# theouterlimitz/Audio-Mastering-Engine

Measured on NVIDIA B200. Metric: audio-sec mastered/sec (x realtime), higher is better.
Workload: dtype f64

## Files before the change

### audio_mastering_engine_b200/csrc/ame.cu

```cuda
#include <algorithm>
#include <cmath>
#include <cstdarg>
#include <cstdio>
#include <cstring>
#include <dlfcn.h>
#include <mutex>
#include <string>
#include <vector>

#include "ame_kernels.cuh"

using namespace ame;

namespace {

thread_local std::string g_err;

int fail(int code, const char *fmt, ...) {
    char buf[512];
    va_list ap;
    va_start(ap, fmt);
    vsnprintf(buf, sizeof buf, fmt, ap);
    va_end(ap);
    g_err = buf;
// ... 114 lines not shown
    std::vector<Slot> slots;
    double *d_energy = nullptr;
    int *d_chain_stats = nullptr;
    long long *d_hist = nullptr;
    int *d_hist_st = nullptr;
    int *d_peak = nullptr;
    unsigned *d_tp = nullptr;
    int *d_lim_stats = nullptr;
    int lim_guess = -1;
    ame_track_result *d_results = nullptr;
    KwJob *d_meter_kw = nullptr;
    GainJob *d_meter_peak = nullptr;
    int32_t *d_meter_tracks = nullptr;
    TrackDev *d_meter_tdev = nullptr;
    double *d_meter_energy = nullptr;
    int *d_meter_sp = nullptr;
    unsigned *d_meter_tp = nullptr;
    ame_loudness *d_loud_out = nullptr;
    ame_loudness *d_loud_any = nullptr;
    cudaStream_t s_in = nullptr, s_out = nullptr;
    std::vector<cudaEvent_t> ev_in, ev_run;
    std::vector<cudaEvent_t> ev_meter;
    bool timing = false;
    int t_step = -1, t_wave = 0;
    std::vector<cudaEvent_t> t_ev;
    std::vector<char> t_used;
    std::vector<cudaEvent_t> tl_ev;
    int tl_waves = 0;
};

namespace {

inline bool t_on(const ame_plan *p) {
    return p->timing && p->t_step >= 0 && p->t_step < kMaxTimedSteps && p->t_wave < kMaxTimedWaves;
}
inline size_t t_slot(const ame_plan *p, int kernel) {
    return ((size_t)p->t_step * kMaxTimedWaves + p->t_wave) * AME_N_KERNELS + kernel;
}
inline void t_begin(ame_plan *p, int kernel, cudaStream_t s) {
    if (t_on(p)) cudaEventRecord(p->t_ev[t_slot(p, kernel) * 2], s);
}
inline void t_end(ame_plan *p, int kernel, cudaStream_t s) {
    if (t_on(p)) {
        cudaEventRecord(p->t_ev[t_slot(p, kernel) * 2 + 1], s);
        p->t_used[t_slot(p, kernel)] = 1;
    }
}

int plan_alloc(ame_plan *p, void **ptr, size_t bytes) {
    *ptr = nullptr;
    if (bytes == 0) return AME_OK;
    cudaError_t e = dev_alloc(ptr, bytes);
    if (e != cudaSuccess) {
        *ptr = nullptr;
        return fail(AME_E_NOMEM, "device allocation of %zu bytes failed: %s", bytes, cudaGetErrorString(e));
    }
    p->allocs.push_back(*ptr);
    return AME_OK;
}

int dmalloc(ame_plan *p, void **ptr, size_t bytes) {
    const int rc = plan_alloc(p, ptr, bytes);
    if (rc == AME_OK) p->ws_bytes += bytes;
    return rc;
}

template <class T>
int upload(ame_plan *p, T **dptr, const std::vector<T> &v) {
    if (int rc = plan_alloc(p, (void **)dptr, v.size() * sizeof(T))) return rc;
    if (!v.empty()) CU(cudaMemcpy(*dptr, v.data(), v.size() * sizeof(T), cudaMemcpyHostToDevice));
    return AME_OK;
}

#define LAUNCH_CHECK(p)                                                                            \
    do {                                                                                           \
        cudaError_t e_ = cudaGetLastError();                                                       \
        if (e_ != cudaSuccess) return fail(AME_E_CUDA, "kernel launch failed: %s (%s:%d)", cudaGetErrorString(e_), __FILE__, __LINE__); \
        ++(p)->launches;                                                                           \
    } while (0)

int check_warmth(const ame_plan *p) {
    for (int t = 0; t < p->n_tracks; ++t)
        if (p->tracks[t].flags & AME_F_WARMTH) {
            const int l = p->tracks[t].warm_lut;
            if (l < 0 || l >= p->n_luts) return fail(AME_E_INVALID, "track %d needs warmth table %d but %d are set", t, l, p->n_luts);
        }
    return AME_OK;
}

struct Bufs {
    const int16_t *in = nullptr;
    int16_t *pre = nullptr, *bands = nullptr, *out = nullptr;
    uint16_t *rms = nullptr, *list = nullptr;
    int *tile_cnt = nullptr, *n_flagged = nullptr;
    GrpRec *grp = nullptr;
    double *att = nullptr;
    int64_t *hist = nullptr;
    int16_t *norm = nullptr;
    long long *lim_last = nullptr;
    LimStore lim_in{}, lim_out{};
    int *lim_need = nullptr;
};

Bufs slot_bufs(ame_plan *p, const Wave &w, const int16_t *d_in, int16_t *d_out) {
    const Slot &sl = p->slots[w.slot];
    Bufs b;
    b.in = d_in; b.out = d_out;
    b.pre = sl.pre - 2 * w.frame_lo;
    b.bands = sl.bands; b.rms = sl.rms; b.list = sl.list; b.tile_cnt = sl.tile_cnt; b.n_flagged = sl.n_flagged;
    b.grp = sl.grp; b.att = sl.att;
    b.norm = sl.norm ? sl.norm - 2 * w.frame_lo : nullptr;
    b.lim_last = sl.lim_last; b.lim_in = sl.lim_in; b.lim_out = sl.lim_out; b.lim_need = sl.lim_need;
    b.hist = (int64_t *)p->d_hist;
    return b;
}

int run_eq(ame_plan *p, const Wave &w, const int16_t *d_in, int16_t *d_pre, cudaStream_t s) {
    if (!w.eq.n) return AME_OK;
    t_begin(p, S_EQ, s);
    if (p->precision == 1)
        k_eq_f32<<<(w.eq.n + 127) / 128, 128, 0, s>>>(p->d_eq_jobs + w.eq.lo, w.eq.n, p->d_tracks, p->d_luts, d_in, d_pre);
    else
        k_eq<<<(w.eq.n + kEqBlock - 1) / kEqBlock, kEqBlock, 0, s>>>(p->d_eq_jobs + w.eq.lo, w.eq.n, p->d_tracks, p->d_luts, d_in, d_pre);
    LAUNCH_CHECK(p);
    t_end(p, S_EQ, s);
    return AME_OK;
}

int run_split(ame_plan *p, const Wave &w, const int16_t *d_pre, int16_t *d_bands, cudaStream_t s) {
    if (!w.split.n) return AME_OK;
    t_begin(p, S_SPLIT, s);
    if (w.xover_uni)
        k_band_split<true><<<(w.split.n + 127) / 128, 128, 0, s>>>(w.xover, p->d_split_jobs + w.split.lo, w.split.n, p->d_tracks, p->d_mb_delta,
                                                                   d_pre, d_bands, p->mb_frames);
    else
        k_band_split<false><<<(w.split.n + 127) / 128, 128, 0, s>>>(w.xover, p->d_split_jobs + w.split.lo, w.split.n, p->d_tracks, p->d_mb_delta,
                                                                    d_pre, d_bands, p->mb_frames);
    LAUNCH_CHECK(p);
    t_end(p, S_SPLIT, s);
    return AME_OK;
}

int chain_lanes(const ame_plan *p, int n_chains) {
    if (p->chain_warps < 0) return 1;
    if (p->chain_warps > 0) return 32 * p->chain_warps;
    if (n_chains * 2 <= p->n_sm) return 256;
    return (n_chains >= p->n_sm && p->slots.size() > 1) ? 64 : 128;
}

int run_compress(ame_plan *p, const Wave &w, const Bufs &b, cudaStream_t s) {
    if (!w.chain.n) return AME_OK;
    t_begin(p, S_FLAG, s);
    int *tile_base = b.tile_cnt + std::max(p->slot_tiles, 1);
    k_window_flag<<<w.wf.n, kWfThreads, 0, s>>>(p->d_wf_jobs + w.wf.lo, b.bands, b.rms, b.tile_cnt, b.grp);
    LAUNCH_CHECK(p);
    k_tile_prefix<<<w.chain.n, kWfThreads, 0, s>>>(p->d_chain_jobs + w.chain.lo, b.tile_cnt, tile_base, b.n_flagged);
    LAUNCH_CHECK(p);
    k_compact<<<(w.wf.n + kWfThreads / 32 - 1) / (kWfThreads / 32), kWfThreads, 0, s>>>(p->d_wf_jobs + w.wf.lo, w.wf.n, b.rms, b.tile_cnt,
                                                                                          tile_base, b.list, b.grp);
    LAUNCH_CHECK(p);
    t_end(p, S_FLAG, s);
    t_begin(p, S_CHAIN, s);
    const int lanes = chain_lanes(p, w.chain.n);
    k_att_chain<<<w.chain.n, std::max(lanes, 32), 0, s>>>(p->d_chain_jobs + w.chain.lo, b.list, b.n_flagged, p->d_tables, b.att, p->mb_frames,
                                            lanes, p->d_chain_stats + 2 * (size_t)w.chain.lo);
    LAUNCH_CHECK(p);
    t_end(p, S_CHAIN, s);
    t_begin(p, S_APPLY, s);
    k_compress_apply<<<(unsigned)((w.seg_hi - w.seg_lo + 3) / 4), 128, 0, s>>>(p->d_mb_chunks + w.mb_chunks.lo, w.mb_chunks.n, w.seg_lo, w.seg_hi,
                                                                                b.bands, b.grp, b.att, b.pre, p->mb_frames);
    LAUNCH_CHECK(p);
    t_end(p, S_APPLY, s);
    return AME_OK;
}

int run_hist(ame_plan *p, const Wave &w, const int16_t *d_pre, int64_t *d_hist, cudaStream_t s) {
    const int nt = w.track_hi - w.track_lo;
    if (nt <= 0) return AME_OK;
    CU(cudaMemsetAsync(p->d_peak + w.track_lo, 0, (size_t)nt * 4, s));
    if (w.kw.n) {
        t_begin(p, S_KW, s);
        if (w.kw_uni)
            k_kweight_energy<true><<<(w.kw.n + 127) / 128, 128, 0, s>>>(w.kw_cfg, p->d_kw_jobs + w.kw.lo, w.kw.n, p->d_tracks, p->d_tdev, d_pre,
                                                                        p->d_energy, p->d_peak);
        else
            k_kweight_energy<false><<<(w.kw.n + 127) / 128, 128, 0, s>>>(w.kw_cfg, p->d_kw_jobs + w.kw.lo, w.kw.n, p->d_tracks, p->d_tdev, d_pre,
                                                                         p->d_energy, p->d_peak);
        LAUNCH_CHECK(p);
        t_end(p, S_KW, s);
    }
    t_begin(p, S_TAIL, s);
    k_tail_peak<<<nt, 128, 0, s>>>(p->d_tracks, p->d_tdev, w.track_lo, w.track_hi, d_pre, p->d_peak);
    LAUNCH_CHECK(p);
    t_end(p, S_TAIL, s);
    CU(cudaMemsetAsync(p->d_tp + w.track_lo, 0, (size_t)nt * 4, s));
    if (w.true_peak && w.gain.n) {
        t_begin(p, S_TP, s);
        k_true_peak<<<w.gain.n, 256, 0, s>>>(p->d_gain_jobs + w.gain.lo, p->d_tracks, d_pre, p->d_tp);
        LAUNCH_CHECK(p);
        t_end(p, S_TP, s);
    }
    t_begin(p, S_HIST, s);
    k_block_hist<<<nt, 256, 0, s>>>(p->d_tdev, w.track_lo, p->d_energy, (long long *)d_hist, p->d_hist_st);
    LAUNCH_CHECK(p);
    t_end(p, S_HIST, s);
    return AME_OK;
}

int run_apply(ame_plan *p, const Wave &w, const int16_t *d_pre, int16_t *d_out, const Bufs &b, cudaStream_t s) {
    int16_t *d_norm = b.norm;
    long long *lim_last = b.lim_last;
    if (!w.gain.n) return AME_OK;
    t_begin(p, S_GAIN, s);
    if (w.limiter) CU(cudaMemsetAsync(lim_last, 0xff, (size_t)w.lim.n * sizeof(long long), s));
    k_apply_gain<<<w.gain.n, 256, 0, s>>>(p->d_gain_jobs + w.gain.lo, p->d_results, p->d_tracks, p->d_tdev, d_pre, d_out, d_norm, lim_last);
    LAUNCH_CHECK(p);
    t_end(p, S_GAIN, s);
    if (w.limiter) {
        t_begin(p, S_LIM, s);
        const GainJob *gj = p->d_lim_jobs + w.lim.lo;
        constexpr int kLimRounds = 2;
        int cap = 64;
        while (cap < p->lim_keep + 2) cap *= 2;
        const size_t smem = lim_smem_bytes(cap);
        for (int round = 0; round <= kLimRounds; ++round) {
            if (round == 0) {
                k_limiter<<<w.lim.n, 256, smem, s>>>(gj, w.lim.n, lim_last, p->d_tracks, d_norm, d_out, b.lim_in, b.lim_out, b.lim_need, 0, cap, p->lim_guess);
                LAUNCH_CHECK(p);
            }
            k_limiter<<<w.lim.n, 32, smem, s>>>(gj, w.lim.n, lim_last, p->d_tracks, d_norm, d_out, b.lim_in, b.lim_out, b.lim_need, round, cap, p->lim_guess);
            LAUNCH_CHECK(p);
            k_lim_verify<<<(w.lim.n + 3) / 4, 128, 0, s>>>(gj, w.lim.n, p->d_tracks, b.lim_in, b.lim_out, b.lim_need,
                                                             p->d_lim_stats + round);
            LAUNCH_CHECK(p);
        }
        k_lim_fallback<<<w.lim.n, 32, smem, s>>>(gj, w.lim.n, p->d_tracks, d_norm, d_out, b.lim_in, b.lim_out, b.lim_need, cap);
        LAUNCH_CHECK(p);
        t_end(p, S_LIM, s);
    }
    return AME_OK;
}

int run_gain(ame_plan *p, const Wave &w, const int16_t *d_pre, const int64_t *d_hist, int16_t *d_out, const Bufs &b, cudaStream_t s) {
    const int nt = w.track_hi - w.track_lo;
    if (nt <= 0) return AME_OK;
    t_begin(p, S_FIN, s);
    k_finalize<<<nt, 128, 0, s>>>(p->d_tracks, w.track_lo, w.track_hi, (const long long *)d_hist, p->d_hist_st, p->d_peak,
                                             p->d_tp, p->d_results);
    LAUNCH_CHECK(p);
    t_end(p, S_FIN, s);
    return run_apply(p, w, d_pre, d_out, b, s);
}

int run_meter(ame_plan *p, const Wave &w, const int16_t *buf, ame_loudness *res, cudaStream_t s) {
    if (!w.meter_tracks.n) return AME_OK;
    const int nt = w.track_hi - w.track_lo;
    CU(cudaMemsetAsync(p->d_meter_sp + w.track_lo, 0, (size_t)nt * 4, s));
    CU(cudaMemsetAsync(p->d_meter_tp + w.track_lo, 0, (size_t)nt * 4, s));
    if (w.meter_kw.n) {
        if (w.kw_uni)
            k_kweight_energy<true><<<(w.meter_kw.n + 127) / 128, 128, 0, s>>>(w.kw_cfg, p->d_meter_kw + w.meter_kw.lo, w.meter_kw.n, p->d_tracks,
                                                                              p->d_meter_tdev, buf, p->d_meter_energy, p->d_meter_sp);
        else
            k_kweight_energy<false><<<(w.meter_kw.n + 127) / 128, 128, 0, s>>>(w.kw_cfg, p->d_meter_kw + w.meter_kw.lo, w.meter_kw.n, p->d_tracks,
                                                                               p->d_meter_tdev, buf, p->d_meter_energy, p->d_meter_sp);
        LAUNCH_CHECK(p);
    }
    if (w.meter_peak.n) {
        k_meter_peak<<<w.meter_peak.n, 256, 0, s>>>(p->d_meter_peak + w.meter_peak.lo, p->d_tracks, buf, p->d_meter_tp, p->d_meter_sp);
        LAUNCH_CHECK(p);
    }
    k_meter_finalize<<<w.meter_tracks.n, 256, 0, s>>>(p->d_meter_tracks + w.meter_tracks.lo, p->d_tracks, p->d_meter_tdev, p->d_meter_energy,
                                                      p->d_meter_sp, p->d_meter_tp, res);
    LAUNCH_CHECK(p);
    return AME_OK;
}

int run_measure(ame_plan *p, const Wave &w, const Bufs &b, cudaStream_t s) {
    int rc;
    if ((rc = run_eq(p, w, b.in, b.pre, s))) return rc;
    if ((rc = run_split(p, w, b.pre, b.bands, s))) return rc;
    if ((rc = run_compress(p, w, b, s))) return rc;
    return run_hist(p, w, b.pre, b.hist, s);
}

int run_chain_of_stages(ame_plan *p, const Wave &w, const Bufs &b, cudaStream_t s) {
    int rc = run_measure(p, w, b, s);
    if (rc) return rc;
    return run_gain(p, w, b.pre, b.hist, b.out, b, s);
}

int drain(ame_plan *p, int rc) {
    (void)p;
    if (rc != AME_OK) cudaDeviceSynchronize();
    return rc;
}

}

extern "C" {

int ame_abi_version(void) { return AME_ABI_VERSION; }
size_t ame_sizeof_track_params(void) { return sizeof(ame_track_params); }
size_t ame_sizeof_track_result(void) { return sizeof(ame_track_result); }
size_t ame_sizeof_plan_options(void) { return sizeof(ame_plan_options); }
size_t ame_sizeof_loudness(void) { return sizeof(ame_loudness); }
const char *ame_last_error(void) { return g_err.c_str(); }
// ... 615 lines not shown
```

### audio_mastering_engine_b200/csrc/ame_kernels.cuh

```cuda
#pragma once
#include <cuda_runtime.h>
#include <stdint.h>
#include "ame_layout.h"

namespace ame {

constexpr unsigned kFull = 0xffffffffu;

__constant__ double c_hist_bounds[1001];
__constant__ double c_hist_energy[1000];

__device__ __forceinline__ uint4 ldg16(const uint4 *p) { return __ldg(p); }

__device__ __forceinline__ double bq_step(const ame_biquad &c, double &z0, double &z1, double x) {
    double y = fma(c.b0, x, z0);
    z0 = fma(-c.a1, y, fma(c.b1, x, z1));
    z1 = fma(-c.a2, y, c.b2 * x);
    return y;
}

__device__ __forceinline__ double i16_to_f64(int x) {
    return __hiloint2double(0x43300000, (int)(0x80000000u ^ (unsigned)x)) - 4503601774854144.0;
}

// ... 144 lines not shown
        }
        if (widen) {
            const float mid = __fmul_rn(__fadd_rn(yl, yr), 0.5f);
            const float side = __fmul_rn(__fmul_rn(__fsub_rn(yl, yr), 0.5f), wfac);
            yl = __fadd_rn(mid, side);
            yr = __fsub_rn(mid, side);
        }
        return pack16(to_pcm_f32(yl), to_pcm_f32(yr));
    };

    const uint4 *src = reinterpret_cast<const uint4 *>(in) + (g0f >> 2);
    uint4 *dst = reinterpret_cast<uint4 *>(pre) + (g0f >> 2);
    uint4 cur = ldg16(src), nxt = make_uint4(0, 0, 0, 0);
    if (g0f + 0 < job.chunk_begin) cur.x = 0;
    if (g0f + 1 < job.chunk_begin) cur.y = 0;
    if (g0f + 2 < job.chunk_begin) cur.z = 0;
    if (n_it > 1) nxt = ldg16(src + 1);
    double lutL[4] = {0, 0, 0, 0}, lutR[4] = {0, 0, 0, 0};
    auto fetch_lut = [&](const uint4 &q, double *l, double *r) {
        const uint32_t w[4] = {q.x, q.y, q.z, q.w};
#pragma unroll
        for (int k = 0; k < 4; ++k) {
            l[k] = __ldg(lut + (int)(int16_t)(w[k] & 0xffffu));
            r[k] = __ldg(lut + (int)(int16_t)(w[k] >> 16));
        }
    };
    if (WARM) fetch_lut(cur, lutL, lutR);
    constexpr int LAG = (SKEW && MASK != 0) ? 1 : 0;
    for (int it = 0; it < n_it + LAG; ++it) {
        uint4 nn = nxt;
        if (it + 2 < n_it) nn = ldg16(src + it + 2);
        double nL[4] = {0, 0, 0, 0}, nR[4] = {0, 0, 0, 0};
        if (WARM) fetch_lut(nxt, nL, nR);
        const int64_t g = g0f + 4 * (int64_t)(it - LAG);
        const uint32_t w[4] = {cur.x, cur.y, cur.z, cur.w};
        uint32_t o[4];
#pragma unroll
        for (int k = 0; k < 4; ++k) o[k] = frame(w[k], lutL[k], lutR[k]);
        if (it < LAG) {
        } else if (g >= job.tile_begin && g + 4 <= f_hi) {
            dst[it - LAG] = make_uint4(o[0], o[1], o[2], o[3]);
        } else {
#pragma unroll
            for (int k = 0; k < 4; ++k)
                if (g + k >= job.tile_begin && g + k < f_hi) reinterpret_cast<uint32_t *>(dst + it - LAG)[k] = o[k];
        }
        cur = nxt; nxt = nn;
#pragma unroll
        for (int k = 0; k < 4; ++k) { lutL[k] = nL[k]; lutR[k] = nR[k]; }
    }
}

#define AME_EQ_KERNEL(NAME, F, SK)                                                                                  \
__global__ void __launch_bounds__(256, 1)                                                                          \
NAME(const TileJob *__restrict__ jobs, int n_jobs, const ame_track_params *__restrict__ tracks,                    \
     const double *__restrict__ luts, const int16_t *__restrict__ in, int16_t *__restrict__ pre) {                 \
    const int j = blockIdx.x * blockDim.x + threadIdx.x;                                                           \
    if (j >= n_jobs) return;                                                                                       \
    const TileJob job = jobs[j];                                                                                   \
    if (job.tile_end <= job.tile_begin) return;                          \
    const ame_track_params *tp = tracks + job.track;                                                               \
    switch (job.variant) {                                                 \
        AME_EQ_CASE(0, F, SK) AME_EQ_CASE(1, F, SK) AME_EQ_CASE(2, F, SK) AME_EQ_CASE(3, F, SK) AME_EQ_CASE(4, F, SK)    \
        AME_EQ_CASE(5, F, SK) AME_EQ_CASE(6, F, SK) AME_EQ_CASE(7, F, SK) AME_EQ_CASE(8, F, SK) AME_EQ_CASE(9, F, SK)    \
        AME_EQ_CASE(10, F, SK) AME_EQ_CASE(11, F, SK) AME_EQ_CASE(12, F, SK) AME_EQ_CASE(13, F, SK) AME_EQ_CASE(14, F, SK) \
        AME_EQ_CASE(15, F, SK)                                                                                     \
    }                                                                                                              \
}
#define AME_EQ_CASE(M, F, SK) case M: eq_tile<M, false, F, SK>(job, tp, luts, in, pre); break; \
                              case M + 16: eq_tile<M, true, F, SK>(job, tp, luts, in, pre); break;
AME_EQ_KERNEL(k_eq, double, false)
AME_EQ_KERNEL(k_eq_f32, float, false)
#undef AME_EQ_CASE
#undef AME_EQ_KERNEL

template <bool UNI>
__global__ void __launch_bounds__(128, 3)
k_band_split(const __grid_constant__ XoverCfg xc, const TileJob *__restrict__ jobs, int n_jobs, const ame_track_params *__restrict__ tracks,
             const int64_t *__restrict__ mb_delta,
             const int16_t *__restrict__ pre, int16_t *__restrict__ bands, int64_t mb_frames) {
    const int j = blockIdx.x * blockDim.x + threadIdx.x;
    if (j >= n_jobs) return;
    const TileJob job = jobs[j];
    const ame_track_params *tp = tracks + job.track;
    const double lb0 = UNI ? xc.lb0 : tp->xlp[0].b0, la10 = UNI ? xc.la10 : tp->xlp[0].a1, la20 = UNI ? xc.la20 : tp->xlp[0].a2,
                 la11 = UNI ? xc.la11 : tp->xlp[1].a1, la21 = UNI ? xc.la21 : tp->xlp[1].a2;
    const double hb0 = UNI ? xc.hb0 : tp->xhp[0].b0, ha10 = UNI ? xc.ha10 : tp->xhp[0].a1, ha20 = UNI ? xc.ha20 : tp->xhp[0].a2,
                 ha11 = UNI ? xc.ha11 : tp->xhp[1].a1, ha21 = UNI ? xc.ha21 : tp->xhp[1].a2;
    const int64_t delta = mb_delta[job.track];
    double zl[8], zr[8];
#pragma unroll
    for (int i = 0; i < 8; ++i) { zl[i] = 0.0; zr[i] = 0.0; }
    int64_t f_lo = job.tile_begin - (int64_t)tp->warm_xover;
    if (f_lo < job.chunk_begin) f_lo = job.chunk_begin;
    const int64_t f_hi = job.tile_end;
    if (f_hi <= f_lo) return;
    const int64_t g0f = f_lo & ~(int64_t)7;
    const int n_it = (int)((f_hi - g0f + 7) >> 3);
    uint32_t *b0 = reinterpret_cast<uint32_t *>(bands) + delta;
    uint32_t *b1 = b0 + mb_frames;
    uint32_t *b2 = b1 + mb_frames;

    auto split = [&](int xm, double *z, int &p0, int &p1, int &p2) {
        const double x = i16_to_unit(xm);
        const double lo = bw_step1<1, double>(la11, la21, z[2], z[3], bw_step<1, double>(lb0, la10, la20, z[0], z[1], x));
        const double hi = bw_step1<-1, double>(ha11, ha21, z[6], z[7], bw_step<-1, double>(hb0, ha10, ha20, z[4], z[5], x));
        const double mid = __dsub_rn(__dsub_rn(x, lo), hi);
        p0 = to_pcm_f64(lo); p1 = to_pcm_f64(mid); p2 = to_pcm_f64(hi);
    };

    const uint4 *src = reinterpret_cast<const uint4 *>(pre) + (g0f >> 2);
    uint4 c0 = ldg16(src), c1 = ldg16(src + 1), n0 = make_uint4(0, 0, 0, 0), n1 = n0;
    {
        uint32_t *cw0 = reinterpret_cast<uint32_t *>(&c0), *cw1 = reinterpret_cast<uint32_t *>(&c1);
#pragma unroll
        for (int k = 0; k < 4; ++k) {
            if (g0f + k < job.chunk_begin) cw0[k] = 0;
            if (g0f + 4 + k < job.chunk_begin) cw1[k] = 0;
        }
    }
    if (n_it > 1) { n0 = ldg16(src + 2); n1 = ldg16(src + 3); }
    for (int it = 0; it < n_it; ++it) {
        uint4 m0 = n0, m1 = n1;
        if (it + 2 < n_it) { m0 = ldg16(src + 2 * it + 4); m1 = ldg16(src + 2 * it + 5); }
        const int64_t g = g0f + 8 * (int64_t)it;
        const uint32_t w[8] = {c0.x, c0.y, c0.z, c0.w, c1.x, c1.y, c1.z, c1.w};
        uint32_t o0[8], o1[8], o2[8];
#pragma unroll
        for (int k = 0; k < 8; ++k) {
            int l0, l1, l2, r0, r1, r2;
            split((int)(int16_t)(w[k] & 0xffffu), zl, l0, l1, l2);
            split((int)(int16_t)(w[k] >> 16), zr, r0, r1, r2);
            o0[k] = pack16(l0, r0); o1[k] = pack16(l1, r1); o2[k] = pack16(l2, r2);
        }
        if (g >= job.tile_begin && g + 8 <= f_hi) {
            uint4 *q0 = reinterpret_cast<uint4 *>(b0 + g), *q1 = reinterpret_cast<uint4 *>(b1 + g), *q2 = reinterpret_cast<uint4 *>(b2 + g);
            q0[0] = make_uint4(o0[0], o0[1], o0[2], o0[3]); q0[1] = make_uint4(o0[4], o0[5], o0[6], o0[7]);
            q1[0] = make_uint4(o1[0], o1[1], o1[2], o1[3]); q1[1] = make_uint4(o1[4], o1[5], o1[6], o1[7]);
            q2[0] = make_uint4(o2[0], o2[1], o2[2], o2[3]); q2[1] = make_uint4(o2[4], o2[5], o2[6], o2[7]);
        } else {
#pragma unroll
            for (int k = 0; k < 8; ++k)
                if (g + k >= job.tile_begin && g + k < f_hi) { b0[g + k] = o0[k]; b1[g + k] = o1[k]; b2[g + k] = o2[k]; }
        }
        c0 = n0; c1 = n1; n0 = m0; n1 = m1;
    }
}

__device__ __forceinline__ unsigned energy_of(uint32_t w) {
    const int l = (int16_t)(w & 0xffffu), r = (int16_t)(w >> 16);
    return (unsigned)(l * l) + (unsigned)(r * r);
}

__device__ __forceinline__ void load8(const uint32_t *__restrict__ p, int64_t idx, int64_t lo, int64_t hi, uint32_t *w) {
    if (idx >= lo && idx + 8 <= hi && ((reinterpret_cast<uintptr_t>(p + idx) & 15) == 0)) {
        const uint4 a = __ldg(reinterpret_cast<const uint4 *>(p + idx));
        const uint4 b = __ldg(reinterpret_cast<const uint4 *>(p + idx) + 1);
        w[0] = a.x; w[1] = a.y; w[2] = a.z; w[3] = a.w; w[4] = b.x; w[5] = b.y; w[6] = b.z; w[7] = b.w;
    } else {
#pragma unroll
        for (int k = 0; k < 8; ++k) w[k] = (idx + k >= lo && idx + k < hi) ? __ldg(p + idx + k) : 0u;
    }
}

__device__ __forceinline__ unsigned isqrt_ratio(unsigned long long s, unsigned n) {
    unsigned r = (unsigned)__fsqrt_rn(__fdividef((float)s, (float)n));
    if ((unsigned long long)r * r * n > s) --r;
    else if ((unsigned long long)(r + 1) * (r + 1) * n <= s) ++r;
    return r;
}

__global__ void __launch_bounds__(kWfThreads)
k_window_flag(const WfJob *__restrict__ jobs, const int16_t *__restrict__ bands, uint16_t *__restrict__ rms,
              int *__restrict__ tile_cnt, GrpRec *__restrict__ grp) {
    __shared__ long long s_scan[kWfThreads / 32];
    __shared__ unsigned long long s_head[kWfThreads / 32];
    __shared__ int s_flag[kWfThreads / 32];
    const WfJob job = jobs[blockIdx.x];
    const uint32_t *bp = reinterpret_cast<const uint32_t *>(bands) + job.plane_off;
    uint16_t *rp = rms + job.plane_off;
    const int64_t n = job.n, t0 = job.tile_begin;
    const int look = job.look;
    const int lane = threadIdx.x & 31, wid = threadIdx.x >> 5;
    const int64_t i0 = t0 + (int64_t)threadIdx.x * 8;
    uint32_t w[8], wo[8];
    load8(bp, i0, 0, n, w);
    load8(bp, i0 - look, 0, n, wo);
    unsigned long long head = 0;
    for (int64_t j = t0 - look + threadIdx.x; j < t0; j += kWfThreads)
        if (j >= 0) head += energy_of(__ldg(bp + j));
#pragma unroll
    for (int d = 16; d > 0; d >>= 1) head += __shfl_xor_sync(kFull, head, d);
    if (lane == 0) s_head[wid] = head;
    long long pre[8];
    long long run = 0;
#pragma unroll
    for (int k = 0; k < 8; ++k) {
        pre[k] = run;
        run += (long long)energy_of(w[k]) - (long long)energy_of(wo[k]);
    }
    long long incl = run;
#pragma unroll
    for (int d = 1; d < 32; d <<= 1) {
        const long long v = __shfl_up_sync(kFull, incl, d);
        if (lane >= d) incl += v;
    }
    if (lane == 31) s_scan[wid] = incl;
    __syncthreads();
    long long base = incl - run;
    unsigned long long h = 0;
#pragma unroll
    for (int q = 0; q < kWfThreads / 32; ++q) {
        if (q < wid) base += s_scan[q];
        h += s_head[q];
    }
    base += (long long)h;
    const unsigned long long thr2 = (unsigned long long)job.thr_i * job.thr_i;
    const bool never = job.thr_i > 32768u;
    uint32_t o[4] = {0, 0, 0, 0};
    unsigned m8 = 0;
    if (t0 >= look && i0 + 8 <= n) {
        const unsigned long long bound = thr2 * (unsigned long long)(2 * look);
#pragma unroll
        for (int k = 0; k < 8; ++k) {
            const unsigned long long s = (unsigned long long)(base + pre[k]);
            unsigned r = 0;
            if (!never && s >= bound) r = isqrt_ratio(s, (unsigned)(2 * look));
            m8 |= (r != 0 ? 1u : 0u) << k;
            o[k >> 1] |= (r & 0xffffu) << ((k & 1) * 16);
        }
    } else {
#pragma unroll
        for (int k = 0; k < 8; ++k) {
            const int64_t i = i0 + k;
            const long long s = base + pre[k];
            const int64_t nfr = i < look ? i : look;
            unsigned r = 0;
            if (!never && i < n && nfr > 0 && (unsigned long long)s >= thr2 * (unsigned long long)(2 * nfr))
                r = isqrt_ratio((unsigned long long)s, (unsigned)(2 * nfr));
            m8 |= (r != 0 ? 1u : 0u) << k;
            o[k >> 1] |= (r & 0xffffu) << ((k & 1) * 16);
        }
    }
    const int cnt = __popc(m8);
    int fincl = cnt;
#pragma unroll
    for (int d = 1; d < 32; d <<= 1) {
        const int v = __shfl_up_sync(kFull, fincl, d);
        if (lane >= d) fincl += v;
    }
    if (lane == 31) s_flag[wid] = fincl;
    const unsigned m1 = __shfl_down_sync(kFull, m8, 1), m2 = __shfl_down_sync(kFull, m8, 2), m3 = __shfl_down_sync(kFull, m8, 3);
    __syncthreads();
    int fbase = 0, total = 0;
#pragma unroll
    for (int q = 0; q < kWfThreads / 32; ++q) {
        if (q < wid) fbase += s_flag[q];
        total += s_flag[q];
    }
    const int rank = fbase + fincl - cnt;
    if ((threadIdx.x & 3) == 0 && i0 < n)
        grp[job.grp_begin + (i0 >> 5)] = GrpRec{m8 | (m1 << 8) | (m2 << 16) | (m3 << 24), (uint32_t)rank};
    if (m8) {
        uint16_t *dp = rp + t0 + rank;
        int slot = 0;
#pragma unroll
        for (int k = 0; k < 8; ++k)
            if (m8 & (1u << k)) dp[slot++] = (uint16_t)((o[k >> 1] >> ((k & 1) * 16)) & 0xffffu);
    }
    if (threadIdx.x == 0) tile_cnt[blockIdx.x] = total;
}

__device__ __forceinline__ double att_update(double att, double m, double inc, double dec, double tau) {
    const long long ia = __double_as_longlong(att);
    const bool above = ia > __double_as_longlong(m);
    const bool rising = ia < __double_as_longlong(tau);
    const double s = att + inc;
    const double d = att - dec;
    const double r = above ? d : m;
    return (rising && !above) ? s : r;
}

struct RmsBlk { uint32_t w[4]; };

__device__ __forceinline__ RmsBlk list_load(const uint16_t *__restrict__ lp, int64_t i, int64_t lim, bool vec) {
    RmsBlk q;
    q.w[0] = q.w[1] = q.w[2] = q.w[3] = 0;
    if (vec && i + 8 <= lim) {
        const uint4 v = __ldg(reinterpret_cast<const uint4 *>(lp + i));
        q.w[0] = v.x; q.w[1] = v.y; q.w[2] = v.z; q.w[3] = v.w;
    } else if (i < lim) {
#pragma unroll
        for (int k = 0; k < 8; ++k)
            if (i + k < lim) q.w[k >> 1] |= (uint32_t)__ldg(lp + i + k) << ((k & 1) * 16);
    }
    return q;
}

__global__ void __launch_bounds__(kWfThreads)
k_tile_prefix(const ChainJob *__restrict__ jobs, const int *__restrict__ tile_cnt, int *__restrict__ tile_base,
              int *__restrict__ n_flagged) {
    __shared__ int s_warp[kWfThreads / 32];
    const ChainJob job = jobs[blockIdx.x];
    const int n_tiles = (int)((job.n + kWfTile - 1) / kWfTile);
    const int t = threadIdx.x, lane = t & 31, wid = t >> 5;
    int carry = 0;
    for (int j0 = 0; j0 < n_tiles; j0 += kWfThreads) {
        const int j = j0 + t;
        const int c = j < n_tiles ? tile_cnt[job.tile0 + j] : 0;
        int incl = c;
#pragma unroll
        for (int d = 1; d < 32; d <<= 1) {
            const int v = __shfl_up_sync(kFull, incl, d);
            if (lane >= d) incl += v;
        }
        if (lane == 31) s_warp[wid] = incl;
        __syncthreads();
        int base = carry, total = 0;
#pragma unroll
        for (int q = 0; q < kWfThreads / 32; ++q) {
            if (q < wid) base += s_warp[q];
            total += s_warp[q];
        }
        if (j < n_tiles) tile_base[job.tile0 + j] = base + incl - c;
        carry += total;
        __syncthreads();
    }
    if (t == 0) n_flagged[blockIdx.x] = carry;
}

__global__ void __launch_bounds__(kWfThreads)
k_compact(const WfJob *__restrict__ jobs, int n_tiles, const uint16_t *__restrict__ rms, const int *__restrict__ tile_cnt,
          const int *__restrict__ tile_base, uint16_t *__restrict__ list, GrpRec *__restrict__ grp) {
    const int lane = threadIdx.x & 31;
    const int tile = blockIdx.x * (kWfThreads / 32) + (threadIdx.x >> 5);
    if (tile >= n_tiles) return;
    const WfJob job = jobs[tile];
    const int cnt = tile_cnt[tile], base = tile_base[tile];
    if (base) {
        const int64_t frames = min((int64_t)kWfTile, job.n - job.tile_begin);
        const int ng = (int)((frames + 31) >> 5);
        GrpRec *gr = grp + job.grp_begin + (job.tile_begin >> 5);
        for (int g = lane; g < ng; g += 32) gr[g].base += (uint32_t)base;
    }
    const uint16_t *rp = rms + job.plane_off + job.tile_begin;
    uint16_t *lp = list + job.plane_off + base;
    for (int j = lane; j < cnt; j += 32) lp[j] = rp[j];
}


__device__ __forceinline__ void list_entries(AttEntry *e, const AttEntry *tbl, const RmsBlk &q) {
#pragma unroll
    for (int k = 0; k < 8; ++k) {
        const unsigned r = (q.w[k >> 1] >> ((k & 1) * 16)) & 0xffffu;
        asm("ld.global.nc.v4.f64 {%0,%1,%2,%3}, [%4];" : "=d"(e[k].m), "=d"(e[k].inc), "=d"(e[k].dec), "=d"(e[k].tau) : "l"(tbl + r));
    }
}

struct SegSum {
    long long margin;
    long long at_p;
    long long lo, hi;
    int64_t p;
    int exp0;
    bool open;
    bool ok;
};

__device__ __forceinline__ void segsum_begin(SegSum &u, double start) {
    u.margin = 0x7fffffffffffffffLL; u.at_p = 0; u.lo = 0; u.hi = -1; u.p = 0;
    u.exp0 = (int)(__double_as_longlong(start) >> 52);
    u.open = true; u.ok = u.exp0 > 0;
}

template <bool DUAL>
__device__ __forceinline__ bool list_step8(const AttEntry *e, double *al, int64_t i, int64_t lim, bool avec, double &a, double &b,
                                           SegSum &u, double &max_m, double &sum_dec) {
    double o[8];
#pragma unroll
    for (int k = 0; k < 8; ++k) {
        if (!DUAL) { max_m = fmax(max_m, e[k].m); sum_dec += e[k].dec; }
        if (DUAL && u.open && i + k < lim) {
            const long long ib = __double_as_longlong(b), im = __double_as_longlong(e[k].m);
            if (ib > im) {
                u.margin = min(u.margin, ib - im);
                const long long id = __double_as_longlong(e[k].dec);
                if (id != 0) {
                    const int ed = (int)(id >> 52);
                    const long long mant = (id & 0xfffffffffffffLL) | (ed ? (1LL << 52) : 0LL);
                    if ((ed ? ed : 1) + (__ffsll(mant) - 1) == u.exp0 - 1) u.ok = false;
                }
                ++u.p;
            } else {
                u.open = false;
                u.at_p = ib; u.lo = __double_as_longlong(e[k].tau); u.hi = im;
                if ((int)(ib >> 52) != u.exp0) u.ok = false;
            }
        }
        b = att_update(b, e[k].m, e[k].inc, e[k].dec, e[k].tau);
        if (DUAL) a = att_update(a, e[k].m, e[k].inc, e[k].dec, e[k].tau);
        o[k] = b;
    }
    if (avec && i + 8 <= lim) {
        double2 *d = reinterpret_cast<double2 *>(al + i);
        d[0] = make_double2(o[0], o[1]); d[1] = make_double2(o[2], o[3]);
        d[2] = make_double2(o[4], o[5]); d[3] = make_double2(o[6], o[7]);
    } else {
#pragma unroll
        for (int k = 0; k < 8; ++k)
            if (i + k < lim) al[i + k] = o[k];
    }
    return DUAL && __double_as_longlong(a) == __double_as_longlong(b);
}

template <bool DUAL>
__device__ __forceinline__ bool list_walk(const uint16_t *lp, const AttEntry *tbl, double *al, int64_t b0, int64_t b1, bool vec,
                                          bool avec, double a, double &b, SegSum &u, double &max_m, double &sum_dec) {
    if (b0 >= b1) return false;
    RmsBlk r0 = list_load(lp, b0, b1, vec), r1 = list_load(lp, b0 + 8, b1, vec);
    AttEntry ea[8], eb[8];
    list_entries(ea, tbl, r0);
    for (int64_t i = b0; i < b1; i += 16) {
        r0 = list_load(lp, i + 16, b1, vec);
// ... 867 lines not shown
```

Measured before the change: 929,600.

## Rewrite window-flag kernel as four-lane per-tile sequential walk

The window-flag kernel used to give each tile a full block of kWfThreads threads, with block-wide scans through shared memory and __syncthreads. It now gives each tile a quad of four lanes that walk the tile in 32-frame groups, using quad shuffles for the scans and prefetching the next groups with 256-bit non-coherent loads where alignment allows. The integer sqrt seed now uses sqrt.approx and is still corrected exactly afterwards. The aim is to drop the block-level synchronisation and shared-memory overhead and to cut thread count per tile, at the cost of much less parallelism per tile and a longer serial walk.

After: 948,400, median of 6. 2.0% higher.

```diff
diff --git a/audio_mastering_engine_b200/csrc/ame.cu b/audio_mastering_engine_b200/csrc/ame.cu
--- a/audio_mastering_engine_b200/csrc/ame.cu
+++ b/audio_mastering_engine_b200/csrc/ame.cu
@@ -290,7 +290,7 @@
     if (!w.chain.n) return AME_OK;
     t_begin(p, S_FLAG, s);
     int *tile_base = b.tile_cnt + std::max(p->slot_tiles, 1);
-    k_window_flag<<<w.wf.n, kWfThreads, 0, s>>>(p->d_wf_jobs + w.wf.lo, b.bands, b.rms, b.tile_cnt, b.grp);
+    k_window_flag<<<(4 * w.wf.n + kWfBlock - 1) / kWfBlock, kWfBlock, 0, s>>>(p->d_wf_jobs + w.wf.lo, w.wf.n, b.bands, b.rms, b.tile_cnt, b.grp);
     LAUNCH_CHECK(p);
     k_tile_prefix<<<w.chain.n, kWfThreads, 0, s>>>(p->d_chain_jobs + w.chain.lo, b.tile_cnt, tile_base, b.n_flagged);
     LAUNCH_CHECK(p);
diff --git a/audio_mastering_engine_b200/csrc/ame_kernels.cuh b/audio_mastering_engine_b200/csrc/ame_kernels.cuh
--- a/audio_mastering_engine_b200/csrc/ame_kernels.cuh
+++ b/audio_mastering_engine_b200/csrc/ame_kernels.cuh
@@ -320,123 +320,160 @@
     return (unsigned)(l * l) + (unsigned)(r * r);
 }
 
-__device__ __forceinline__ void load8(const uint32_t *__restrict__ p, int64_t idx, int64_t lo, int64_t hi, uint32_t *w) {
-    if (idx >= lo && idx + 8 <= hi && ((reinterpret_cast<uintptr_t>(p + idx) & 15) == 0)) {
-        const uint4 a = __ldg(reinterpret_cast<const uint4 *>(p + idx));
-        const uint4 b = __ldg(reinterpret_cast<const uint4 *>(p + idx) + 1);
-        w[0] = a.x; w[1] = a.y; w[2] = a.z; w[3] = a.w; w[4] = b.x; w[5] = b.y; w[6] = b.z; w[7] = b.w;
-    } else {
-#pragma unroll
-        for (int k = 0; k < 8; ++k) w[k] = (idx + k >= lo && idx + k < hi) ? __ldg(p + idx + k) : 0u;
-    }
-}
-
 __device__ __forceinline__ unsigned isqrt_ratio(unsigned long long s, unsigned n) {
-    unsigned r = (unsigned)__fsqrt_rn(__fdividef((float)s, (float)n));
+    float q;
+    asm("sqrt.approx.f32 %0, %1;" : "=f"(q) : "f"(__fdividef((float)s, (float)n)));
+    unsigned r = (unsigned)q;
     if ((unsigned long long)r * r * n > s) --r;
     else if ((unsigned long long)(r + 1) * (r + 1) * n <= s) ++r;
     return r;
 }
 
-__global__ void __launch_bounds__(kWfThreads)
-k_window_flag(const WfJob *__restrict__ jobs, const int16_t *__restrict__ bands, uint16_t *__restrict__ rms,
+constexpr int kWfBlock = 128;
+
+struct WfState {
+    unsigned long long s;
+    unsigned m;
+    int cnt, base;
+};
+
+__device__ __forceinline__ void wf_walk_frames(const uint32_t *__restrict__ bp, uint16_t *__restrict__ dp, GrpRec *__restrict__ gp,
+                                               int64_t a, int64_t b, int64_t t0, int64_t te, int look,
+                                               unsigned long long thr2, bool never, WfState &st) {
+    for (int64_t i = a; i < b; ++i) {
+        const unsigned e = energy_of(__ldg(bp + i));
+        const unsigned eo = i >= look ? energy_of(__ldg(bp + i - look)) : 0u;
+        const int64_t nfr = i < look ? i : look;
+        if (!never && nfr > 0 && st.s >= thr2 * (unsigned long long)(2 * nfr)) {
+            dp[st.cnt++] = (uint16_t)isqrt_ratio(st.s, (unsigned)(2 * nfr));
+            st.m |= 1u << (i & 31);
+        }
+        st.s = st.s + e - eo;
+        if ((i & 31) == 31 || i + 1 == te) {
+            gp[(i - t0) >> 5] = GrpRec{st.m, (uint32_t)st.base};
+            st.base = st.cnt;
+            st.m = 0;
+        }
+    }
+}
+
+struct Frames8 { uint32_t w[8]; };
+
+template <bool WIDE>
+__device__ __forceinline__ Frames8 wf_load(const uint32_t *p) {
+    Frames8 f;
+    if (WIDE) {
+        asm("ld.global.nc.v8.u32 {%0,%1,%2,%3,%4,%5,%6,%7}, [%8];"
+            : "=r"(f.w[0]), "=r"(f.w[1]), "=r"(f.w[2]), "=r"(f.w[3]), "=r"(f.w[4]), "=r"(f.w[5]), "=r"(f.w[6]), "=r"(f.w[7])
+            : "l"(p));
+    } else {
+        const uint4 a = ldg16(reinterpret_cast<const uint4 *>(p)), b = ldg16(reinterpret_cast<const uint4 *>(p) + 1);
+        f.w[0] = a.x; f.w[1] = a.y; f.w[2] = a.z; f.w[3] = a.w; f.w[4] = b.x; f.w[5] = b.y; f.w[6] = b.z; f.w[7] = b.w;
+    }
+    return f;
+}
+
+template <bool WM, bool WO>
+__device__ __forceinline__ void wf_walk_groups(const uint32_t *__restrict__ p, const uint32_t *__restrict__ po,
+                                               uint16_t *__restrict__ dp, GrpRec *__restrict__ gq, int n_grp, int look,
+                                               unsigned long long bound, int q, unsigned qm, WfState &st) {
+    long long d = (long long)(st.s - bound);
+    const uint32_t *pl = p + 8 * q, *pol = po + 8 * q;
+    Frames8 c = wf_load<WM>(pl), n = wf_load<WM>(pl + 32 * min(1, n_grp - 1)), co = wf_load<WO>(pol);
+    for (int g = 0; g < n_grp; ++g) {
+        const int gn = min(g + 2, n_grp - 1), go = min(g + 1, n_grp - 1);
+        const Frames8 nn = wf_load<WM>(pl + 32 * gn), no = wf_load<WO>(pol + 32 * go);
+        long long df[8], sum = 0;
+#pragma unroll
+        for (int k = 0; k < 8; ++k) { df[k] = (long long)energy_of(c.w[k]) - (long long)energy_of(co.w[k]); sum += df[k]; }
+        long long incl = sum, v;
+        v = __shfl_up_sync(qm, incl, 1, 4); if (q >= 1) incl += v;
+        v = __shfl_up_sync(qm, incl, 2, 4); if (q >= 2) incl += v;
+        long long e = d + incl - sum;
+        const long long e0 = e;
+        unsigned m8 = 0;
+#pragma unroll
+        for (int k = 0; k < 8; ++k) { m8 |= (e >= 0 ? 1u : 0u) << k; e += df[k]; }
+        d += __shfl_sync(qm, incl, 3, 4);
+        const int cn = __popc(m8);
+        int ci = cn, w;
+        w = __shfl_up_sync(qm, ci, 1, 4); if (q >= 1) ci += w;
+        w = __shfl_up_sync(qm, ci, 2, 4); if (q >= 2) ci += w;
+        if (m8) {
+            int r = st.cnt + ci - cn;
+            e = e0;
+#pragma unroll
+            for (int k = 0; k < 8; ++k) {
+                if (m8 & (1u << k)) dp[r++] = (uint16_t)isqrt_ratio((unsigned long long)e + bound, (unsigned)(2 * look));
+                e += df[k];
+            }
+        }
+        unsigned m = m8 << (8 * q);
+        m |= __shfl_xor_sync(qm, m, 1, 4);
+        m |= __shfl_xor_sync(qm, m, 2, 4);
+        if (q == 0) gq[g] = GrpRec{m, (uint32_t)st.cnt};
+        st.cnt += __shfl_sync(qm, ci, 3, 4);
+        c = n; n = nn; co = no;
+    }
+    st.s = (unsigned long long)d + bound;
+    st.base = st.cnt;
+}
+
+__global__ void __launch_bounds__(kWfBlock)
+k_window_flag(const WfJob *__restrict__ jobs, int n_jobs, const int16_t *__restrict__ bands, uint16_t *__restrict__ rms,
               int *__restrict__ tile_cnt, GrpRec *__restrict__ grp) {
-    __shared__ long long s_scan[kWfThreads / 32];
-    __shared__ unsigned long long s_head[kWfThreads / 32];
-    __shared__ int s_flag[kWfThreads / 32];
-    const WfJob job = jobs[blockIdx.x];
+    const int t = blockIdx.x * blockDim.x + threadIdx.x;
+    const int j = t >> 2, q = t & 3;
+    if (j >= n_jobs) return;
+    const unsigned qm = 0xfu << (threadIdx.x & 28);
+    const WfJob job = jobs[j];
     const uint32_t *bp = reinterpret_cast<const uint32_t *>(bands) + job.plane_off;
-    uint16_t *rp = rms + job.plane_off;
-    const int64_t n = job.n, t0 = job.tile_begin;
+    const int64_t t0 = job.tile_begin, te = min(t0 + (int64_t)kWfTile, job.n);
     const int look = job.look;
-    const int lane = threadIdx.x & 31, wid = threadIdx.x >> 5;
-    const int64_t i0 = t0 + (int64_t)threadIdx.x * 8;
-    uint32_t w[8], wo[8];
-    load8(bp, i0, 0, n, w);
-    load8(bp, i0 - look, 0, n, wo);
-    unsigned long long head = 0;
-    for (int64_t j = t0 - look + threadIdx.x; j < t0; j += kWfThreads)
-        if (j >= 0) head += energy_of(__ldg(bp + j));
-#pragma unroll
-    for (int d = 16; d > 0; d >>= 1) head += __shfl_xor_sync(kFull, head, d);
-    if (lane == 0) s_head[wid] = head;
-    long long pre[8];
-    long long run = 0;
-#pragma unroll
-    for (int k = 0; k < 8; ++k) {
-        pre[k] = run;
-        run += (long long)energy_of(w[k]) - (long long)energy_of(wo[k]);
-    }
-    long long incl = run;
-#pragma unroll
-    for (int d = 1; d < 32; d <<= 1) {
-        const long long v = __shfl_up_sync(kFull, incl, d);
-        if (lane >= d) incl += v;
-    }
-    if (lane == 31) s_scan[wid] = incl;
-    __syncthreads();
-    long long base = incl - run;
-    unsigned long long h = 0;
-#pragma unroll
-    for (int q = 0; q < kWfThreads / 32; ++q) {
-        if (q < wid) base += s_scan[q];
-        h += s_head[q];
-    }
-    base += (long long)h;
+    uint16_t *dp = rms + job.plane_off + t0;
+    GrpRec *gp = grp + job.grp_begin + (t0 >> 5);
     const unsigned long long thr2 = (unsigned long long)job.thr_i * job.thr_i;
     const bool never = job.thr_i > 32768u;
-    uint32_t o[4] = {0, 0, 0, 0};
-    unsigned m8 = 0;
-    if (t0 >= look && i0 + 8 <= n) {
-        const unsigned long long bound = thr2 * (unsigned long long)(2 * look);
-#pragma unroll
-        for (int k = 0; k < 8; ++k) {
-            const unsigned long long s = (unsigned long long)(base + pre[k]);
-            unsigned r = 0;
-            if (!never && s >= bound) r = isqrt_ratio(s, (unsigned)(2 * look));
-            m8 |= (r != 0 ? 1u : 0u) << k;
-            o[k >> 1] |= (r & 0xffffu) << ((k & 1) * 16);
-        }
-    } else {
-#pragma unroll
-        for (int k = 0; k < 8; ++k) {
-            const int64_t i = i0 + k;
-            const long long s = base + pre[k];
-            const int64_t nfr = i < look ? i : look;
-            unsigned r = 0;
-            if (!never && i < n && nfr > 0 && (unsigned long long)s >= thr2 * (unsigned long long)(2 * nfr))
-                r = isqrt_ratio((unsigned long long)s, (unsigned)(2 * nfr));
-            m8 |= (r != 0 ? 1u : 0u) << k;
-            o[k >> 1] |= (r & 0xffffu) << ((k & 1) * 16);
-        }
-    }
-    const int cnt = __popc(m8);
-    int fincl = cnt;
-#pragma unroll
-    for (int d = 1; d < 32; d <<= 1) {
-        const int v = __shfl_up_sync(kFull, fincl, d);
-        if (lane >= d) fincl += v;
-    }
-    if (lane == 31) s_flag[wid] = fincl;
-    const unsigned m1 = __shfl_down_sync(kFull, m8, 1), m2 = __shfl_down_sync(kFull, m8, 2), m3 = __shfl_down_sync(kFull, m8, 3);
-    __syncthreads();
-    int fbase = 0, total = 0;
-#pragma unroll
-    for (int q = 0; q < kWfThreads / 32; ++q) {
-        if (q < wid) fbase += s_flag[q];
-        total += s_flag[q];
-    }
-    const int rank = fbase + fincl - cnt;
-    if ((threadIdx.x & 3) == 0 && i0 < n)
-        grp[job.grp_begin + (i0 >> 5)] = GrpRec{m8 | (m1 << 8) | (m2 << 16) | (m3 << 24), (uint32_t)rank};
-    if (m8) {
-        uint16_t *dp = rp + t0 + rank;
-        int slot = 0;
-#pragma unroll
-        for (int k = 0; k < 8; ++k)
-            if (m8 & (1u << k)) dp[slot++] = (uint16_t)((o[k >> 1] >> ((k & 1) * 16)) & 0xffffu);
-    }
-    if (threadIdx.x == 0) tile_cnt[blockIdx.x] = total;
+    WfState st{0, 0, 0, 0};
+    const int64_t h = max(t0 - look, (int64_t)0);
+    const int64_t ha = h - (int64_t)((reinterpret_cast<uintptr_t>(bp + h) >> 2) & 7);
+    for (int64_t x = ha + 8 * q; x < t0; x += 32) {
+        if (x >= h && x + 8 <= t0) {
+            const Frames8 f = wf_load<true>(bp + x);
+#pragma unroll
+            for (int k = 0; k < 8; ++k) st.s += energy_of(f.w[k]);
+        } else {
+#pragma unroll
+            for (int k = 0; k < 8; ++k)
+                if (x + k >= h && x + k < t0) st.s += energy_of(__ldg(bp + x + k));
+        }
+    }
+    st.s += __shfl_xor_sync(qm, st.s, 1, 4);
+    st.s += __shfl_xor_sync(qm, st.s, 2, 4);
+    const int64_t f1 = t0 + ((te - t0) & ~(int64_t)31);
+    const int64_t f0 = min(max(t0, ((int64_t)look + 31) & ~(int64_t)31), f1);
+    const uint32_t *p = bp + f0, *po = bp + f0 - look;
+    const uintptr_t am = reinterpret_cast<uintptr_t>(p), ao = reinterpret_cast<uintptr_t>(po);
+    const bool fast = f0 < f1 && ((am | ao) & 15) == 0;
+    if (q == 0) wf_walk_frames(bp, dp, gp, t0, fast ? f0 : f1, t0, te, look, thr2, never, st);
+    if (fast) {
+        st.s = __shfl_sync(qm, st.s, 0, 4);
+        st.cnt = st.base = __shfl_sync(qm, st.cnt, 0, 4);
+        const int n_grp = (int)((f1 - f0) >> 5);
+        const unsigned long long bound = never ? (1ull << 62) : thr2 * (unsigned long long)(2 * look);
+        GrpRec *gq = gp + ((f0 - t0) >> 5);
+        if (am & 31) {
+            if (ao & 31) wf_walk_groups<false, false>(p, po, dp, gq, n_grp, look, bound, q, qm, st);
+            else wf_walk_groups<false, true>(p, po, dp, gq, n_grp, look, bound, q, qm, st);
+        } else {
+            if (ao & 31) wf_walk_groups<true, false>(p, po, dp, gq, n_grp, look, bound, q, qm, st);
+            else wf_walk_groups<true, true>(p, po, dp, gq, n_grp, look, bound, q, qm, st);
+        }
+    }
+    if (q == 0) {
+        wf_walk_frames(bp, dp, gp, f1, te, t0, te, look, thr2, never, st);
+        tile_cnt[j] = st.cnt;
+    }
 }
 
 __device__ __forceinline__ double att_update(double att, double m, double inc, double dec, double tau) {
```
